# yjhuangcd/FI-ODE

Measured on AMD Instinct MI355X. Metric: CIFAR-10 train-step images/sec (B=128, h_sample=256) at 1/2/4/8 MI355X, higher is better.
Workload: dtype f32; 1 GPU; hipGraph replay: BASELINE configs[1]: train step of README.md:27 at epoch 20 with train_ode (rk4, step_size 0.1, t_max=1: 10 steps / 40 train-mode f-evals, backprop through the stages; loss_ode portion 0.2) + the Lyapunov loss (B=128, h_sample_size=256 -> 204 uniform + 52 correct-cone rows/image), KWLarge-Cayley backbone + Adam; global_batch=128, h_sample_size=256, rows_per_rank=32768, parallelism=dp1

## Files before the change

### fi-ode_amd/csrc/sconv.hip

```cpp
#include <hip/hip_runtime.h>
#include <stdint.h>

#include "common.h"
#include "fft.h"
#include "fiode.h"

namespace {

typedef float2 c32;
constexpr int BT_F = 16;
constexpr int BT_I = 8;
#ifndef SCONV_NTF8
#define SCONV_NTF8 512
#endif
#ifndef SCONV_NTF16
#define SCONV_NTF16 512
#endif
#ifndef SCONV_NTF32
#define SCONV_NTF32 512
#endif
#ifndef SCONV_NTF32S
#define SCONV_NTF32S 512
#endif
#ifndef SCONV_NTI8
// ... 37 lines not shown
  const c32* Y;
  const float* bias;
  float* y;
  uint8_t* code_out;
  const float* xn;
  const float* mu;
  const float* sd;
  const c32* Q;
  const c32* Xq;
};

__device__ __forceinline__ int64_t act_index(const SArgs& a, int h, int w, int c, int b) {
  return (((int64_t)h * a.n + w) * a.C + c) * a.B + b;
}
__device__ __forceinline__ int64_t nchw_index(const SArgs& a, int h, int w, int c, int b) {
  return (((int64_t)b * a.C + c) * a.n + h) * a.n + w;
}
__device__ __forceinline__ int64_t code_index(const SArgs& a, int h, int w, int c0, int b) {
  const int half = a.C >> 1;
  return a.nchw ? (((int64_t)b * half + c0) * a.n + h) * a.n + w : (((int64_t)h * a.n + w) * half + c0) * a.B + b;
}
__device__ __forceinline__ int64_t raw_index(const SArgs& a, int h, int w, int c, int b) {
  const int cr = c >> 2, dh = (c >> 1) & 1, dw = c & 1, C4 = a.C >> 2, n2 = 2 * a.n;
  return (((int64_t)(2 * h + dh) * n2 + (2 * w + dw)) * C4 + cr) * a.B + b;
}

constexpr int pad_is(int n, int bt, bool inv) {
  return inv ? (n == 8 ? 76 : n == 16 ? 276 : (bt == 4 ? 1064 : 1060))
             : n == 8 ? (bt == 4 ? 72 : 74) : n == 16 ? (bt == 4 ? 280 : 274)
                                                      : (bt == 4 ? 1064 : bt == 8 ? 1060 : 1058);
}
constexpr int pad_zs(int n, int bt, bool inv) {
  return inv ? (n == 8 ? 42 : n == 16 ? 146 : (bt == 4 ? 548 : 546))
             : n == 8 ? (bt == 4 ? 44 : 41) : n == 16 ? (bt == 4 ? 148 : 145)
                                                      : (bt == 4 ? 548 : bt == 8 ? 546 : 545);
}
template <int N, int BT, bool INV>
struct Geo {
  static constexpr int H = N / 2 + 1;
  static constexpr int RS = N + 1;
  static constexpr int IS = pad_is(N, BT, INV);
  static constexpr int ZS = pad_zs(N, BT, INV);
  static_assert(IS >= N * RS && ZS >= N * H, "image strides");
};

template <int N, int BT>
struct FGeo {
  typedef Geo<N, BT, false> g;
  static constexpr int H = g::H;
  static constexpr int ZS = g::ZS;
  static constexpr int CS = BT * ZS;
  static constexpr int NT = nthreads<N, BT, false>();
  __device__ static int pix(int ch, int bt, int h) { return 2 * (ch * CS + bt * ZS + h * H); }
};

template <int N, int BT, int NCH>
__device__ __forceinline__ void rfft2_inplace(const SArgs& a, int c0, int c1, int b0, c32* Z) {
  typedef FGeo<N, BT> G;
  constexpr int H = G::H, NT = G::NT;
  const float* img = reinterpret_cast<const float*>(Z);
  const int tid = threadIdx.x;
  for (int row = tid; row < NCH * BT * N; row += NT) {
    const int ch = row / (BT * N), r = row - ch * (BT * N);
    const int bt = r % BT, h = r / BT;
    const float* src = img + G::pix(ch, bt, h);
    c32 x[N];
#pragma unroll
    for (int w = 0; w < N; ++w) x[w] = make_float2(src[w], 0.f);
    fiode_fft::fft_reg<N, false>(x);
    c32* dst = Z + ch * G::CS + bt * G::ZS + h * H;
#pragma unroll
    for (int kb = 0; kb < H; ++kb) dst[kb] = x[kb];
  }
  __syncthreads();
  for (int col = tid; col < NCH * BT * H; col += NT) {
    const int ch = col / (BT * H), r = col - ch * (BT * H);
    const int bt = r % BT, kb = r / BT;
    const c32* cp = Z + ch * G::CS + bt * G::ZS + kb;
    c32 x[N];
#pragma unroll
    for (int h = 0; h < N; ++h) x[h] = cp[h * H];
    fiode_fft::fft_reg<N, false>(x);
    const int b = b0 + bt, c = ch ? c1 : c0;
    if (b < a.B) {
#pragma unroll
      for (int ka = 0; ka < N; ++ka) a.X[((int64_t)(ka * H + kb) * a.C + c) * a.B + b] = x[ka];
    }
  }
}

template <int N, int BT>
__global__ void __launch_bounds__((nthreads<N, BT, false>())) k_sconv_rfft2(SArgs a) {
  typedef FGeo<N, BT> G;
  constexpr int NT = G::NT;
  constexpr int NL = BT * N * N;
  constexpr int TR = (NL + NT - 1) / NT;
  __shared__ c32 Z[2 * G::CS];
  float* img = reinterpret_cast<float*>(Z);
  const int b0 = blockIdx.y * BT, tid = threadIdx.x;
  if (a.gy) {
    const int half = a.C >> 1, c0 = blockIdx.x, c1 = c0 + half;
#pragma unroll
    for (int t = 0; t < TR; ++t) {
      const int idx = tid + t * NT;
      if (idx < NL) {
        const int bt = a.nchw ? idx / (N * N) : idx % BT;
        const int hw = a.nchw ? idx % (N * N) : idx / BT, h = hw / N, w = hw % N;
        const int b = min(b0 + bt, a.B - 1);
        const uint8_t code = a.code[code_index(a, h, w, c0, b)];
        const float gmx = a.gy[a.nchw ? nchw_index(a, h, w, c0, b) : act_index(a, h, w, c0, b)];
        const float gmn = a.gy[a.nchw ? nchw_index(a, h, w, c1, b) : act_index(a, h, w, c1, b)];
        const bool in = b0 + bt < a.B;
        img[G::pix(0, bt, h) + w] = in ? gs_grad(gmx, gmn, code, true) : 0.f;
        img[G::pix(1, bt, h) + w] = in ? gs_grad(gmx, gmn, code, false) : 0.f;
      }
    }
// ... 12 lines not shown
        const int b = min(b0 + bt, a.B - 1);
        float v = a.xn[(((int64_t)b * a.C + c) * N + h) * N + w] - m;
        if (a.sd) v = v / sdv;
        img[G::pix(0, bt, h) + w] = b0 + bt < a.B ? v : 0.f;
      }
    }
  } else if (a.ds) {
#pragma unroll
    for (int t = 0; t < TR; ++t) {
      const int idx = tid + t * NT;
      if (idx < NL) {
        const int bt = idx % BT, hw = idx / BT, h = hw / N, w = hw % N;
        const int b = min(b0 + bt, a.B - 1);
        const float v = a.x[raw_index(a, h, w, c, b)];
        img[G::pix(0, bt, h) + w] = b0 + bt < a.B ? v : 0.f;
      }
    }
  } else {
#pragma unroll
    for (int t = 0; t < TR; ++t) {
      const int idx = tid + t * NT;
      if (idx < NL) {
        const int bt = idx % BT, hw = idx / BT, h = hw / N, w = hw % N;
        const int b = min(b0 + bt, a.B - 1);
        const float v = a.x[act_index(a, h, w, c, b)];
        img[G::pix(0, bt, h) + w] = b0 + bt < a.B ? v : 0.f;
      }
    }
  }
  __syncthreads();
  rfft2_inplace<N, BT, 1>(a, c, c, b0, Z);
}

template <int N>
struct IGeo {
  typedef Geo<N, bt_inv<N>(), true> g;
  static constexpr int BTI = bt_inv<N>();
  static constexpr int H = g::H;
  static constexpr int ZS = g::ZS;
  static constexpr int CS = BTI * ZS;
  static constexpr int NT = nthreads<N, BTI, true>();
  __device__ static int pix(int ch, int bt, int h) { return 2 * (ch * CS + bt * ZS + h * H); }
};

template <int N, int NCH, int KQ>
__device__ __forceinline__ void irfft2_inplace(const SArgs& a, int c0, int c1, int b0, c32* Ys) {
  typedef IGeo<N> G;
  constexpr int BTI = G::BTI, H = G::H, NT = G::NT;
  constexpr int NL = NCH * BTI * N * H;
  constexpr int TR = (NL + NT - 1) / NT;
  const int tid = threadIdx.x;
  if constexpr (KQ == 0) {
#pragma unroll
    for (int t = 0; t < TR; ++t) {
      const int idx = tid + t * NT;
      if (idx < NL) {
        const int ch = idx / (BTI * N * H), r = idx - ch * (BTI * N * H);
        const int bt = r % BTI, f = r / BTI;
        const int b = min(b0 + bt, a.B - 1);
        const c32 v = a.Y[((int64_t)f * a.C + (ch ? c1 : c0)) * a.B + b];
        Ys[ch * G::CS + bt * G::ZS + f] = b0 + bt < a.B ? v : make_float2(0.f, 0.f);
      }
    }
  } else {
    constexpr int NL1 = BTI * N * H;
    constexpr int TR1 = (NL1 + NT - 1) / NT;
#pragma unroll
    for (int t = 0; t < TR1; ++t) {
      const int idx = tid + t * NT;
      if (idx < NL1) {
        const int bt = idx % BTI, f = idx / BTI;
        const int b = min(b0 + bt, a.B - 1);
        const c32* xq = a.Xq + (int64_t)f * KQ * a.B + b;
        c32 xk[KQ], qk[NCH][KQ];
#pragma unroll
        for (int k = 0; k < KQ; ++k) xk[k] = xq[(int64_t)k * a.B];
#pragma unroll
        for (int ch = 0; ch < NCH; ++ch) {
          const c32* q = a.Q + ((int64_t)f * a.C + (ch ? c1 : c0)) * KQ;
#pragma unroll
          for (int k = 0; k < KQ; ++k) qk[ch][k] = q[k];
        }
#pragma unroll
        for (int ch = 0; ch < NCH; ++ch) {
          c32 v = make_float2(0.f, 0.f);
#pragma unroll
          for (int k = 0; k < KQ; ++k) {
            v.x += qk[ch][k].x * xk[k].x - qk[ch][k].y * xk[k].y;
            v.y += qk[ch][k].x * xk[k].y + qk[ch][k].y * xk[k].x;
          }
          Ys[ch * G::CS + bt * G::ZS + f] = b0 + bt < a.B ? v : make_float2(0.f, 0.f);
        }
      }
// ... 44 lines not shown
  const int b0 = blockIdx.y * BTI, tid = threadIdx.x;
  if (a.gs) {
    const int half = a.C >> 1, c0 = blockIdx.x, c1 = c0 + half;
    irfft2_inplace<N, 2, KQ>(a, c0, c1, b0, Ys);
    const float bb0 = a.bias ? a.bias[c0] : 0.f, bb1 = a.bias ? a.bias[c1] : 0.f;
    for (int idx = tid; idx < BTI * N * N; idx += NT) {
      const int bt = a.nchw ? idx / (N * N) : idx % BTI;
      const int hw = a.nchw ? idx % (N * N) : idx / BTI, h = hw / N, w = hw % N;
      const int b = b0 + bt;
      if (b >= a.B) continue;
      const float p = o[G::pix(0, bt, h) + w] + bb0, q = o[G::pix(1, bt, h) + w] + bb1;
      a.y[a.nchw ? nchw_index(a, h, w, c0, b) : act_index(a, h, w, c0, b)] = fmaxf(p, q);
      a.y[a.nchw ? nchw_index(a, h, w, c1, b) : act_index(a, h, w, c1, b)] = fminf(p, q);
      a.code_out[code_index(a, h, w, c0, b)] = p > q ? GS_GT : (p < q ? GS_LT : GS_EQ);
    }
    (void)half;
  } else {
    const int c = blockIdx.x;
    irfft2_inplace<N, 1, KQ>(a, c, c, b0, Ys);
    const float bb = a.bias ? a.bias[c] : 0.f;
    for (int idx = tid; idx < BTI * N * N; idx += NT) {
      const int bt = a.nchw ? idx / (N * N) : idx % BTI;
      const int hw = a.nchw ? idx % (N * N) : idx / BTI, h = hw / N, w = hw % N;
      const int b = b0 + bt;
      if (b >= a.B) continue;
      const float v = o[G::pix(0, bt, h) + w] + bb;
      if (a.ds) a.y[raw_index(a, h, w, c, b)] = v;
      else if (a.nchw) a.y[nchw_index(a, h, w, c, b)] = v;
      else a.y[act_index(a, h, w, c, b)] = v;
    }
  }
}

int check(const fiode_sconv_config* cfg, SArgs& a) {
  if (!cfg) return FIODE_EINVAL;
  a = SArgs{};
  a.n = cfg->n;
  a.C = cfg->C;
  a.B = cfg->B;
  a.ds = cfg->downsample ? 1 : 0;
  a.nchw = cfg->nchw ? 1 : 0;
  if ((a.n != 8 && a.n != 16 && a.n != 32) || a.C < 1 || a.B < 1) return FIODE_ESHAPE;
  if (a.nchw && a.ds) return FIODE_ESHAPE;
  if (a.ds && (a.C & 3)) return FIODE_ESHAPE;
  a.H = a.n / 2 + 1;
  return FIODE_OK;
}

}

extern "C" int fiode_sconv_rfft2(void* stream, const fiode_sconv_config* cfg, const float* x, const float* gy,
                                 const uint8_t* code, void* X) {
  SArgs a;
  int rc = check(cfg, a);
  if (rc) return rc;
  if (!X || (!x && !gy) || (gy && (!code || (a.C & 1) || a.ds))) return FIODE_EINVAL;
  a.x = x;
  a.gy = gy;
  a.code = code;
  a.X = (c32*)X;
  hipStream_t st = (hipStream_t)stream;
  const bool small = (int64_t)a.C * ((a.B + BT_F - 1) / BT_F) < 256;
  const int bt = small ? 4 : a.n == 32 ? SCONV_BTF32 : BT_F;
  const dim3 grid(gy ? a.C / 2 : a.C, (a.B + bt - 1) / bt);
  if (a.n == 8) {
    if (small) hipLaunchKernelGGL((k_sconv_rfft2<8, 4>), grid, dim3(nthreads<8, 4, false>()), 0, st, a);
// ... 59 lines not shown
  a.bias = bias;
  a.y = y;
  a.code_out = code_out;
  return FIODE_OK;
}

}

extern "C" int fiode_sconv_irfft2(void* stream, const fiode_sconv_config* cfg, const void* Y, const float* bias,
                                  int32_t groupsort, float* y, uint8_t* code_out) {
  SArgs a;
  const int rc = irfft2_common(cfg, bias, groupsort, y, code_out, a);
  if (rc) return rc;
  if (!Y) return FIODE_EINVAL;
  a.Y = (const c32*)Y;
  const hipError_t e = launch_irfft2<0>(a, (hipStream_t)stream);
  return e == hipSuccess ? FIODE_OK : FIODE_EHIP + (int)e;
}

extern "C" int fiode_sconv_irfft2_qx(void* stream, const fiode_sconv_config* cfg, const void* Q, const void* X,
                                     int32_t K, const float* bias, int32_t groupsort, float* y, uint8_t* code_out) {
  SArgs a;
  const int rc = irfft2_common(cfg, bias, groupsort, y, code_out, a);
  if (rc) return rc;
  if (K < 1 || K > 4) return FIODE_ESHAPE;
  if (!Q || !X) return FIODE_EINVAL;
  a.Q = (const c32*)Q;
  a.Xq = (const c32*)X;
  hipStream_t st = (hipStream_t)stream;
  const hipError_t e = K == 1 ? launch_irfft2<1>(a, st) : K == 2 ? launch_irfft2<2>(a, st)
                     : K == 3 ? launch_irfft2<3>(a, st) : launch_irfft2<4>(a, st);
  return e == hipSuccess ? FIODE_OK : FIODE_EHIP + (int)e;
}
```

### fi-ode_amd/fiode_amd/_lib.py

```python
from __future__ import annotations

import ctypes as ct
import os
import pathlib

_HERE = pathlib.Path(__file__).resolve().parent
LIB_PATH = pathlib.Path(os.environ.get("FIODE_LIB", _HERE / "libfiode.so"))

FIODE_SAMPLER_GIVEN, FIODE_SAMPLER_COMPOSITE, FIODE_SAMPLER_DECISION_BOUNDARY, FIODE_SAMPLER_TRAJECTORY = 0, 1, 2, 3
FIODE_DROPOUT_OFF, FIODE_DROPOUT_GIVEN, FIODE_DROPOUT_PHILOX = 0, 1, 2
FIODE_ACT_RELU, FIODE_ACT_GROUPSORT = 0, 1

class FiodeLibraryError(RuntimeError):
    pass


class FiodeError(RuntimeError):
    pass


_fp = ct.POINTER(ct.c_float)
_vp = ct.c_void_p


# ... 166 lines not shown
        "fiode_ode_nll": (ct.c_int, [_vp, ct.c_int32, _vp, _vp, _vp, _vp]),
        "fiode_ode_loss_mix": (ct.c_int, [_vp, ct.c_int32, _vp, _vp, _vp, ct.c_float, _vp, _vp, _vp]),
        "fiode_small_cayley_forward": (ct.c_int, [_vp, ct.c_int32, ct.c_int32, ct.c_int32, _vp, _vp, _vp, _vp, _vp]),
        "fiode_small_cayley_backward": (ct.c_int, [_vp, ct.c_int32, ct.c_int32, ct.c_int32, _vp, _vp, _vp, _vp, _vp,
                                                   _vp, _vp]),
        "fiode_dense_cayley_prep": (ct.c_int, [_vp, ct.POINTER(DenseConfig), _vp, _vp, _vp, _vp, _vp]),
        "fiode_dense_norm_workspace_bytes": (ct.c_size_t, [ct.POINTER(DenseConfig)]),
        "fiode_dense_norm_partials": (ct.c_int, [_vp, ct.POINTER(DenseConfig), _vp, _vp, ct.c_size_t]),
        "fiode_dense_cayley_prep_normed": (ct.c_int, [_vp, ct.POINTER(DenseConfig), _vp, _vp, _vp, _vp, _vp, _vp]),
        "fiode_dense_norm_partials_clear": (ct.c_int, [_vp, ct.POINTER(DenseConfig), _vp, _vp, ct.c_size_t, _vp,
                                                       ct.c_size_t, ct.c_size_t]),
        "fiode_dense_inverse_flag_bytes": (ct.c_size_t, [ct.c_int32]),
        "fiode_dense_cayley_inverse": (ct.c_int, [_vp, ct.POINTER(DenseConfig), _vp, _vp, _vp, _vp, _vp, _vp, _vp,
                                                  _vp, ct.c_size_t]),
        "fiode_dense_cayley_finish": (ct.c_int, [_vp, ct.POINTER(DenseConfig), _vp, _vp, _vp, _vp, _vp]),
        "fiode_dense_cayley_ginv": (ct.c_int, [_vp, ct.POINTER(DenseConfig), _vp, _vp, _vp, _vp, _vp]),
        "fiode_dense_cayley_h": (ct.c_int, [_vp, ct.POINTER(DenseConfig), _vp, _vp, _vp]),
        "fiode_dense_cayley_workspace_bytes": (ct.c_size_t, [ct.POINTER(DenseConfig)]),
        "fiode_dense_cayley_grad": (ct.c_int, [_vp, ct.POINTER(DenseConfig), _vp, _vp, _vp, _vp, _vp, _vp, _vp, _vp,
                                               _vp, ct.c_size_t]),
        "fiode_dense_gemm": (ct.c_int, [_vp, ct.c_int32, ct.c_int32, ct.c_int32, ct.c_int32, _vp, _vp, _vp]),
        "fiode_gemm_splits": (ct.c_int32, [ct.POINTER(GemmDesc)]),
        "fiode_gemm_counter_bytes": (ct.c_size_t, [ct.POINTER(GemmDesc)]),
        "fiode_gemm_workspace_bytes": (ct.c_size_t, [ct.POINTER(GemmDesc)]),
        "fiode_gemm": (ct.c_int, [_vp, ct.POINTER(GemmDesc), _vp, _vp, _vp, _vp, _vp, ct.c_size_t]),
        "fiode_gemm_pair_workspace_bytes": (ct.c_size_t, [ct.POINTER(GemmDesc), ct.POINTER(GemmDesc)]),
        "fiode_gemm_pair": (ct.c_int, [_vp, ct.POINTER(GemmDesc), _vp, _vp, _vp, _vp, ct.POINTER(GemmDesc), _vp, _vp,
                                       _vp, _vp, _vp, ct.c_size_t]),
        "fiode_sconv_rfft2": (ct.c_int, [_vp, ct.POINTER(SconvConfig), _vp, _vp, _vp, _vp]),
        "fiode_sconv_irfft2": (ct.c_int, [_vp, ct.POINTER(SconvConfig), _vp, _vp, ct.c_int32, _vp, _vp]),
        "fiode_sconv_rfft2_nchw": (ct.c_int, [_vp, ct.POINTER(SconvConfig), _vp, _vp, _vp, _vp]),
        "fiode_sconv_irfft2_qx": (ct.c_int, [_vp, ct.POINTER(SconvConfig), _vp, _vp, ct.c_int32, _vp, ct.c_int32,
                                             _vp, _vp]),
        "fiode_cgemm": (ct.c_int, [_vp, ct.c_int32, ct.c_int32, ct.c_int32, ct.c_int32, ct.c_int32, ct.c_int32, _vp,
                                   _vp, _vp, _vp]),
        "fiode_spectral_workspace_bytes": (ct.c_size_t, [ct.POINTER(SpectralConfig)]),
        "fiode_spectral_cayley_forward": (ct.c_int, [_vp, ct.POINTER(SpectralConfig), _vp, _vp, _vp, _vp, _vp,
                                                     ct.c_size_t]),
        "fiode_spectral_cayley_backward": (ct.c_int, [_vp, ct.POINTER(SpectralConfig), _vp, _vp, _vp, _vp, _vp, _vp,
                                                      _vp, ct.c_size_t]),
        "fiode_adam_step": (ct.c_int, [_vp, ct.POINTER(AdamConfig), _vp, _vp, _vp, _vp, _vp, _vp,
                                       ct.POINTER(StepGuard)]),
        "fiode_step_guard_flag": (ct.c_int, [_vp, ct.POINTER(StepGuard), _vp]),
        "fiode_error_string": (ct.c_char_p, [ct.c_int]),
        "fiode_abi_version": (ct.c_int, []),
    }
    for name, (res, args) in sig.items():
        if not hasattr(lib, name) and "FIODE_LIB" in os.environ:
            continue
        fn = getattr(lib, name)
        fn.restype = res
        fn.argtypes = args
    return lib


_LIB = None


def lib():
    global _LIB
    if _LIB is None:
        lb = _load()
        v = lb.fiode_abi_version()
        if v != ABI_VERSION:
            raise FiodeLibraryError(f"{LIB_PATH}: ABI version {v}, this package binds {ABI_VERSION} "
                                    "(stale build: run `make -C fi-ode_amd/csrc`)")
# ... 9 lines not shown
```

### fi-ode_amd/fiode_amd/cayley.py

```python
from __future__ import annotations

import ctypes as ct
import math
from typing import Optional

import torch
import torch.nn as nn
import torch.nn.functional as F

from .streams import current, fork, join, prefetch, run_on, shared, take


_BLOCK = 128


def _block_inverse(M: torch.Tensor) -> torch.Tensor:
    from . import ops
    n = M.shape[-1]
    if n > 64 and M.dtype == torch.float32 and M.is_cuda:
        if M.dim() == 2:
            return ops.block_inverse(M)
        return ops.block_inverse(M.reshape(-1, n, n)).reshape(M.shape)
    if n <= _BLOCK:
        return ops.batched_inverse(M)
# ... 466 lines not shown
    @staticmethod
    def backward(ctx, gQ):
        from . import ops
        weight, alpha, inv, ws = ctx.saved_tensors
        gw, ga = ops.spectral_cayley_backward(gQ.contiguous(), weight.detach(), alpha.detach(), ctx.n, inv, ws)
        return gw, ga.reshape(alpha.shape), None


class _SpectralCayleyStoredFn(torch.autograd.Function):

    @staticmethod
    def forward(ctx, weight, alpha, n: int, store: dict):
        ctx.save_for_backward(weight, alpha)
        ctx.store, ctx.n = store, n
        return store["Q"].detach()

    @staticmethod
    def backward(ctx, gQ):
        from . import ops
        weight, alpha = ctx.saved_tensors
        st = ctx.store
        gw, ga = ops.spectral_cayley_backward(gQ.contiguous(), weight.detach(), alpha.detach(), ctx.n, st["inv"],
                                              st["ws"])
        ga = ga.reshape(alpha.shape)
        hook = st.get("on_grads")
        if hook is not None:
            hook(gw, ga)
        return gw, ga, None, None


class _SpectralConvFn(torch.autograd.Function):

    @staticmethod
    def forward(ctx, x, Q, bias, n: int, downsample: bool, groupsort: bool, norm=None, nchw_out: bool = False):
        from . import ops
        nf, cout, cin = Q.shape
        if norm is not None:
            B = x.shape[0]
            X = ops.sconv_rfft2_nchw(x.detach(), norm[0], norm[1], n)
        else:
            B = x.shape[-1]
            X = ops.sconv_rfft2(x.detach(), n, cin, B, downsample=downsample)
        bd = None if bias is None else bias.detach()
        if cin <= SCONV_QX_MAX_K and not downsample:
            y, code = ops.sconv_irfft2_qx(Q.detach(), X, n, B, bias=bd, groupsort=groupsort, nchw=nchw_out)
        else:
            y, code = ops.sconv_irfft2(ops.cgemm(Q.detach(), X), n, cout, B, bias=bd, groupsort=groupsort,
                                       nchw=nchw_out)
        ctx.save_for_backward(X, Q, code)
        ctx.cfg = (n, downsample, groupsort, bias is not None, cin, cout, B)
        ctx.nchw_out = nchw_out
        return y

    @staticmethod
    def backward(ctx, gy):
        from . import ops
        X, Q, code = ctx.saved_tensors
        n, downsample, groupsort, has_bias, cin, cout, B = ctx.cfg
        gy = gy.contiguous()
        if groupsort:
            G = ops.sconv_rfft2(None, n, cout, B, gy=gy, code=code, nchw=ctx.nchw_out)
        else:
            G = ops.sconv_rfft2(gy, n, cout, B)
        gx = gQ = gb = None
        need_x, need_q, need_b = ctx.needs_input_grad[0], ctx.needs_input_grad[1], has_bias and ctx.needs_input_grad[2]
        wq = None
        if need_q:
            key = (n, str(G.device))
            wq = _SPECTRAL_GRAD_WEIGHTS.get(key)
            if wq is None:
                kb = torch.arange(n // 2 + 1, device=G.device)
                w = torch.where((kb == 0) | (kb == n // 2), 1.0, 2.0) / float(n * n)
                wq = _SPECTRAL_GRAD_WEIGHTS[key] = w.repeat(n).reshape(-1, 1, 1)

        def wgrad():
            if need_q and CONV_WGRAD_LIB:
                gq = torch.matmul(G, X.mH) * wq
            else:
                gq = ops.cgemm(G, X, conj_trans_b=True, scale=wq.reshape(-1)) if need_q else None
            gbias = G[0].real.sum(-1) if need_b else None
            return gq, gbias
        side = _head_stream(G.device) if (G.is_cuda and need_x and (need_q or need_b)) else None
        branch = fork(side, wgrad, reads=(G, X))
        if need_x:
            gx, _ = ops.sconv_irfft2(_q_h_g(Q, G), n, cin, B, downsample=downsample)
        (gQ, gb), = join(branch)
        return gx, gQ, gb, None, None, None, None, None


_SPECTRAL_GRAD_WEIGHTS = {}
CONV_WGRAD_LIB = True
SCONV_QX_MAX_K = 4


def _q_h_g(Q, G):
    from . import ops
    return ops.cgemm(Q.detach(), G, conj_trans_a=True)




class CayleyConv(nn.Conv2d):

    def __init__(self, in_channels: int, out_channels: int, kernel_size: int, stride: int = 1, bias: bool = True):
        self.downsample = stride == 2
        super().__init__(in_channels * (4 if self.downsample else 1), out_channels, kernel_size, stride=1,
                         padding=kernel_size // 2, bias=bias)
        self.alpha = nn.Parameter(torch.ones(1))
        self._alpha_init = False
        self.fused = True
        self._fused_shapes = {}
        self._shift = {}
        self._n = None
        self._pre = None
        self._store = None

    def _load_from_state_dict(self, *args, **kw):
        super()._load_from_state_dict(*args, **kw)
        self._alpha_init = True

# ... 55 lines not shown
            n = self._n
            self._pre = prefetch(stream, lambda: self.spectral_weight(n, self.weight.device))

    def _take_spectral(self, n: int, device) -> torch.Tensor:
        st = self._store
        if st is not None and self.training and st["n"] == n and torch.is_grad_enabled():
            Q = run_on(current().conv_stream(self),
                       lambda: _SpectralCayleyStoredFn.apply(self.weight, self.alpha, n, st))
            self._pre = None
            return Q
        if self._pre is not None and self.training and self._n == n:
            Q = take(self._pre)
        else:
            Q = self.spectral_weight(n, device)
        self._pre = None
        self._n = n
        return Q

    def forward(self, x: torch.Tensor) -> torch.Tensor:
        if self.downsample:
            b, c, h, w = x.shape
            x = x.reshape(b, c, h // 2, 2, w // 2, 2).permute(0, 1, 3, 5, 2, 4).reshape(b, c * 4, h // 2, w // 2)
        cout, cin = self.weight.shape[:2]
        B, _, n, _ = x.shape
        nf = n * (n // 2 + 1)
        xf = torch.fft.rfft2(x).permute(2, 3, 1, 0).reshape(nf, cin, B)
        Q = self._take_spectral(n, x.device)
        yf = (Q @ xf).reshape(n, n // 2 + 1, cout, B)
        y = torch.fft.irfft2(yf.permute(3, 2, 0, 1), s=(n, n))
        if self.bias is not None:
            y = y + self.bias[:, None, None]
        return y

    def forward_hwcb_fused(self, x: torch.Tensor, groupsort: bool, nchw_out: bool = False) -> torch.Tensor:
        n = x.shape[0] // 2 if self.downsample else x.shape[0]
        Q = self._take_spectral(n, x.device)
        return _SpectralConvFn.apply(x, Q, self.bias, n, self.downsample, groupsort, None,
                                     bool(nchw_out and groupsort))

    def forward_nchw_fused(self, x: torch.Tensor, mu: torch.Tensor, sd, groupsort: bool) -> torch.Tensor:
        n = x.shape[-1]
        Q = self._take_spectral(n, x.device)
        return _SpectralConvFn.apply(x, Q, self.bias, n, False, groupsort, (mu, sd))

    def forward_hwcb(self, x: torch.Tensor) -> torch.Tensor:
        if self.downsample:
            h, w, c, b = x.shape
            x = x.reshape(h // 2, 2, w // 2, 2, c, b).permute(0, 2, 4, 1, 3, 5).reshape(h // 2, w // 2, c * 4, b)
        cout, cin = self.weight.shape[:2]
        n, _, _, B = x.shape
        nf = n * (n // 2 + 1)
        xf = torch.fft.rfft2(x, dim=(0, 1)).reshape(nf, cin, B)
        Q = self._take_spectral(n, x.device)
        yf = Q @ xf
        if self.bias is not None:
            yf[0] += (float(n * n) * self.bias)[:, None]
        return torch.fft.irfft2(yf.reshape(n, n // 2 + 1, cout, B), s=(n, n), dim=(0, 1))
```

### fi-ode_amd/fiode_amd/models.py

```python
from __future__ import annotations

from typing import Optional, Sequence

import torch
import torch.nn as nn

from .cayley import CayleyConv, CayleyLinear, GroupSort, linear_head


class Normalize(nn.Module):

    def __init__(self, mu: Sequence[float], std: Optional[Sequence[float]]):
        super().__init__()
        self.register_buffer("mu", torch.tensor(list(mu), dtype=torch.float32).view(-1, 1, 1))
        self.register_buffer("std", None if std is None else torch.tensor(list(std), dtype=torch.float32).view(-1, 1, 1))

    fused_hwcb = True

    def forward(self, x):
        if self.fused_hwcb and x.is_cuda and x.dtype == torch.float32 and x.dim() == 4 and not x.requires_grad:
            from . import _lib as L, ops
            B, C, H, W = x.shape
            xc = x.contiguous()
            y = torch.empty((H, W, C, B), dtype=torch.float32, device=x.device)
            mu = self.mu.reshape(-1).contiguous()
            sd = None if self.std is None else self.std.reshape(-1).contiguous()
            L.check(L.lib().fiode_normalize_hwcb(ops._stream(x.device), B, C, H, W, xc.data_ptr(), mu.data_ptr(),
                                                 None if sd is None else sd.data_ptr(), y.data_ptr()),
                    "fiode_normalize_hwcb")
            return y.permute(3, 2, 0, 1)
        if self.std is not None:
            return (x - self.mu) / self.std
        return x - self.mu


class KWLargeConcat(nn.Module):

    def __init__(self, out_dim: int = 10, act: str = "GroupSort", w: int = 1):
        super().__init__()
        act_fn = GroupSort if act == "GroupSort" else nn.ReLU
        self.model = nn.Sequential(
            CayleyConv(3, 32 * w, 3), act_fn(),
            CayleyConv(32 * w, 32 * w, 3, stride=2), act_fn(),
            CayleyConv(32 * w, 64 * w, 3), act_fn(),
            CayleyConv(64 * w, 64 * w, 3, stride=2), act_fn(),
            nn.Flatten(),
            CayleyLinear(4096 * w, 512 * w), act_fn(),
            CayleyLinear(512 * w, 512), act_fn(),
            CayleyLinear(512, out_dim),
        )

        self.spatial_major = True
        self.fused_transforms = True
        self.nchw_last = True

    def can_take_nchw(self, x) -> bool:
        m = self.model[0]
        return (self.spatial_major and self.fused_transforms and x.is_cuda and x.dtype == torch.float32
                and x.dim() == 4 and not x.requires_grad and isinstance(m, CayleyConv) and not m.downsample
                and x.shape[-1] == x.shape[-2] and x.shape[-1] in (8, 16, 32))

    def forward(self, x, norm=None):
        if not (self.spatial_major and x.is_cuda):
            return self.model(x)
        mods = list(self.model)
        i = 0
        nconv = 0
        if norm is not None:
            if getattr(self, "after_conv_hook", None) is not None:
                self.after_conv_hook(-1)
            gs = isinstance(mods[1], GroupSort)
            h = mods[0].forward_nchw_fused(x, norm[0], norm[1], gs)
            i = 2 if gs else 1
            if getattr(self, "after_conv_hook", None) is not None:
                self.after_conv_hook(0)
            nconv = 1
        else:
            h = x.permute(2, 3, 1, 0).contiguous()
            if getattr(self, "after_conv_hook", None) is not None:
                self.after_conv_hook(-1)
        nchw = False
        while not isinstance(mods[i], nn.Flatten):
            m = mods[i]
            if isinstance(m, CayleyConv):
                gs = i + 1 < len(mods) and isinstance(mods[i + 1], GroupSort)
                if self.fused_transforms and h.shape[0] // (2 if m.downsample else 1) <= 32:
                    nchw = bool(self.nchw_last and gs and i + 2 < len(mods) and isinstance(mods[i + 2], nn.Flatten))
                    h = m.forward_hwcb_fused(h, gs, nchw_out=nchw)
                    i += 2 if gs else 1
                    if getattr(self, "after_conv_hook", None) is not None:
                        self.after_conv_hook(nconv)
                    nconv += 1
                    continue
                h = m.forward_hwcb(h)
                if getattr(self, "after_conv_hook", None) is not None:
                    self.after_conv_hook(nconv)
                nconv += 1
            elif isinstance(m, GroupSort):
                h = m(h, channel_dim=2)
            else:
                h = m(h)
            i += 1
        h = h.reshape(h.shape[0], -1) if nchw else h.permute(3, 2, 0, 1).reshape(h.shape[3], -1)
        return linear_head(mods[i + 1:], h)


class NormalizedBackbone(nn.Sequential):

    fused_input = True

    def forward(self, x):
        norm, net = self[0], self[1]
        if (self.fused_input and len(self) == 2 and isinstance(norm, Normalize) and isinstance(net, KWLargeConcat)
                and norm.fused_hwcb and net.can_take_nchw(x)):
            return net(x.contiguous(), norm=(norm.mu, norm.std))
        return super().forward(x)


def make_ortho_KWLarge_Concat(n_in_channels=3, n_outputs=10, mu=(0.485, 0.456, 0.406), std=(0.225, 0.225, 0.225),
                              out_dim=10, act="GroupSort"):
    return NormalizedBackbone(Normalize(mu, std), KWLargeConcat(out_dim=out_dim, act=act))
# ... 45 lines not shown
```

### fi-ode_amd/fiode_amd/ops.py

```python
from __future__ import annotations

import ctypes as ct
from dataclasses import dataclass
from typing import Dict, Optional

import torch

from . import _lib as L

C, M, X = 10, 128, 10
WEIGHT_KEYS = ("Q1", "b1", "Qx", "bx", "Q2", "b2", "Q3", "b3")
WEIGHT_SHAPES = {"Q1": (M, C), "b1": (M,), "Qx": (M, X), "bx": (M,), "Q2": (M, M), "b2": (M,),
                 "Q3": (C, M), "b3": (C,)}


@dataclass
class DynCfg:
    alpha_1: float = 100.0
    alpha_2: float = 20.0
    sigma_1: float = 0.02
    scale_nominal: bool = True
    dropout: float = 0.5
    qp_max_iter: int = 30
    qp_tol: float = 1e-4
# ... 638 lines not shown
        bias = _need(bias.detach(), "bias", (C,), torch.float32, dev)
    if nchw and downsample:
        raise ValueError("sconv_irfft2: nchw and downsample together")
    shape = (2 * n, 2 * n, C // 4, B) if downsample else ((B, C, n, n) if nchw else (n, n, C, B))
    y = torch.empty(shape, dtype=torch.float32, device=dev)
    code = (torch.empty((B, C // 2, n, n) if nchw else (n, n, C // 2, B), dtype=torch.uint8, device=dev)
            if groupsort else None)
    cfg = L.SconvConfig(n, C, B, int(bool(downsample)), int(bool(nchw)))
    L.check(L.lib().fiode_sconv_irfft2(_stream(dev), ct.byref(cfg), Y.data_ptr(), _ptr(bias), int(bool(groupsort)),
                                       y.data_ptr(), _ptr(code)), "fiode_sconv_irfft2")
    return y, code


def sconv_irfft2_qx(Q: torch.Tensor, X: torch.Tensor, n: int, B: int, bias: Optional[torch.Tensor] = None,
                    groupsort: bool = False, nchw: bool = False):
    dev = X.device
    nf = n * (n // 2 + 1)
    if Q.dim() != 3 or Q.shape[0] != nf:
        raise ValueError(f"sconv_irfft2_qx: Q {tuple(Q.shape)} is not [{nf}, C, K]")
    C, K = Q.shape[1], Q.shape[2]
    Q = _need(Q.detach(), "Q", (nf, C, K), torch.complex64, dev)
    X = _need(X.detach(), "X", (nf, K, B), torch.complex64, dev)
    if bias is not None:
        bias = _need(bias.detach(), "bias", (C,), torch.float32, dev)
    y = torch.empty((B, C, n, n) if nchw else (n, n, C, B), dtype=torch.float32, device=dev)
    code = (torch.empty((B, C // 2, n, n) if nchw else (n, n, C // 2, B), dtype=torch.uint8, device=dev)
            if groupsort else None)
    cfg = L.SconvConfig(n, C, B, 0, int(bool(nchw)))
    L.check(L.lib().fiode_sconv_irfft2_qx(_stream(dev), ct.byref(cfg), Q.data_ptr(), X.data_ptr(), K, _ptr(bias),
                                          int(bool(groupsort)), y.data_ptr(), _ptr(code)), "fiode_sconv_irfft2_qx")
    return y, code


def cgemm(A: torch.Tensor, B: torch.Tensor, conj_trans_a: bool = False, conj_trans_b: bool = False,
          scale: Optional[torch.Tensor] = None) -> torch.Tensor:
    dev = B.device
    if A.dim() != 3 or B.dim() != 3 or A.dtype != torch.complex64 or B.dtype != torch.complex64:
        raise ValueError(f"cgemm: complex64 [F, ., .] operands, got {tuple(A.shape)} {A.dtype}, "
                         f"{tuple(B.shape)} {B.dtype}")
    if conj_trans_a and conj_trans_b:
        raise ValueError("cgemm: conj_trans_a and conj_trans_b together are not supported")
    F = B.shape[0]
    K, N = (B.shape[2], B.shape[1]) if conj_trans_b else (B.shape[1], B.shape[2])
    M, ka = (A.shape[2], A.shape[1]) if conj_trans_a else (A.shape[1], A.shape[2])
    if A.shape[0] != F or ka != K or A.device != dev:
        raise ValueError(f"cgemm: A {tuple(A.shape)} does not match B {tuple(B.shape)}")
    if scale is not None:
        scale = _need(scale.detach().reshape(-1), "scale", (F,), torch.float32, dev)
    A = A.contiguous()
    B = B.contiguous()
    C = torch.empty((F, M, N), dtype=torch.complex64, device=dev)
    L.check(L.lib().fiode_cgemm(_stream(dev), F, M, N, K, int(bool(conj_trans_a)), int(bool(conj_trans_b)),
                                _ptr(scale), A.data_ptr(), B.data_ptr(), C.data_ptr()), "fiode_cgemm")
    return C


def _mat_layout(X: torch.Tensor):
    R, Cn = X.shape[-2], X.shape[-1]
    s0, s1 = X.stride(-2), X.stride(-1)
    if (s1 == 1 or Cn == 1) and (s0 >= Cn or R == 1):
        return 0, max(s0 if R > 1 else Cn, Cn, 1)
    if (s0 == 1 or R == 1) and (s1 >= R or Cn == 1):
        return 1, max(s1 if Cn > 1 else R, R, 1)
    return None


# ... 208 lines not shown
```

### include/fiode.h

```cpp
#ifndef FIODE_H_
#define FIODE_H_

#include <stddef.h>
#include <stdint.h>

#ifdef __cplusplus
extern "C" {
#endif

#define FIODE_ABI_VERSION 5

#if defined(__GNUC__)
#define FIODE_API __attribute__((visibility("default")))
#else
#define FIODE_API
#endif

enum {
  FIODE_OK = 0,
  FIODE_EINVAL = 1,
  FIODE_ESHAPE = 2,
  FIODE_EWORKSPACE = 3,
  FIODE_EHIP = 100
};
// ... 261 lines not shown
  int32_t trans_a, trans_b;
  int64_t lda, ldb, ldc;
  int64_t stride_a, stride_b, stride_c;
  float alpha, beta;
  int32_t split_k;
  int32_t max_workgroups;
} fiode_gemm_desc;
FIODE_API int32_t fiode_gemm_splits(const fiode_gemm_desc* d);
FIODE_API size_t fiode_gemm_counter_bytes(const fiode_gemm_desc* d);
FIODE_API size_t fiode_gemm_workspace_bytes(const fiode_gemm_desc* d);
FIODE_API int fiode_gemm(void* stream, const fiode_gemm_desc* d, const float* A, const float* B, const float* bias,
                         float* C, void* workspace, size_t workspace_bytes);
FIODE_API size_t fiode_gemm_pair_workspace_bytes(const fiode_gemm_desc* d0, const fiode_gemm_desc* d1);
FIODE_API int fiode_gemm_pair(void* stream, const fiode_gemm_desc* d0, const float* A0, const float* B0,
                              const float* bias0, float* C0, const fiode_gemm_desc* d1, const float* A1,
                              const float* B1, const float* bias1, float* C1, void* workspace,
                              size_t workspace_bytes);

typedef struct fiode_sconv_config {
  int32_t n;
  int32_t C;
  int32_t B;
  int32_t downsample;
  int32_t nchw;
} fiode_sconv_config;
FIODE_API int fiode_sconv_rfft2(void* stream, const fiode_sconv_config* cfg, const float* x, const float* gy,
                                const uint8_t* code, void* X);
FIODE_API int fiode_sconv_rfft2_nchw(void* stream, const fiode_sconv_config* cfg, const float* x, const float* mu,
                                     const float* std, void* X);
FIODE_API int fiode_sconv_irfft2(void* stream, const fiode_sconv_config* cfg, const void* Y, const float* bias,
                                 int32_t groupsort, float* y, uint8_t* code_out);
FIODE_API int fiode_sconv_irfft2_qx(void* stream, const fiode_sconv_config* cfg, const void* Q, const void* X,
                                    int32_t K, const float* bias, int32_t groupsort, float* y, uint8_t* code_out);

FIODE_API int fiode_cgemm(void* stream, int32_t F, int32_t M, int32_t N, int32_t K, int32_t conj_trans_a,
                          int32_t conj_trans_b, const float* scale, const void* A, const void* B, void* C);

typedef struct fiode_spectral_config {
  int32_t cout, cin;
  int32_t ks;
  int32_t n;
} fiode_spectral_config;

FIODE_API size_t fiode_spectral_workspace_bytes(const fiode_spectral_config* cfg);
FIODE_API int fiode_spectral_cayley_forward(void* stream, const fiode_spectral_config* cfg, const float* weight,
                                            const float* alpha, void* Q, void* inv, void* workspace,
                                            size_t workspace_bytes);
FIODE_API int fiode_spectral_cayley_backward(void* stream, const fiode_spectral_config* cfg, const float* weight,
                                             const float* alpha, const void* gQ, const void* inv,
                                             float* grad_weight, float* grad_alpha, void* workspace,
                                             size_t workspace_bytes);

#define FIODE_ADAM_MAX_TENSORS 64
#define FIODE_GUARD_MAX_STATUS 4
typedef struct fiode_step_guard {
  const float* flag;
  const float* loss;
  const int32_t* status[FIODE_GUARD_MAX_STATUS];
  int32_t* skipped;
} fiode_step_guard;
FIODE_API int fiode_step_guard_flag(void* stream, const fiode_step_guard* guard, float* flag_out);

typedef struct fiode_adam_config {
  int32_t n_tensors;
  int32_t decoupled;
  int32_t maximize;
// ... 19 lines not shown
```

Baseline: 105,900 images/s.

## Fuse irfft2+GroupSort+next-layer rfft2 at spectral conv boundaries

Adds boundary kernels that take one layer's spectral output, run the inverse FFT, bias and GroupSort, then apply the next layer's forward FFT (optionally with a space-to-depth downsample) in a single kernel, keeping activations in the spectral domain between consecutive Cayley convs. A matching backward kernel fuses irfft2 of the incoming gradient, the GroupSort gradient and the rfft2. The model's forward path routes eligible conv/GroupSort/conv chains through these kernels, and the backward pass skips the spatial transform when the input was already spectral. This removes the spatial-domain activation round trips through global memory and some launches, at the cost of heavier shared-memory kernels with new tile sizes and more complex autograd plumbing.

```diff
diff --git a/fi-ode_amd/csrc/sconv.hip b/fi-ode_amd/csrc/sconv.hip
--- a/fi-ode_amd/csrc/sconv.hip
+++ b/fi-ode_amd/csrc/sconv.hip
@@ -93,7 +93,7 @@
 }
 constexpr int pad_zs(int n, int bt, bool inv) {
   return inv ? (n == 8 ? 42 : n == 16 ? 146 : (bt == 4 ? 548 : 546))
-             : n == 8 ? (bt == 4 ? 44 : 41) : n == 16 ? (bt == 4 ? 148 : 145)
+             : n == 8 ? (bt == 4 ? 44 : bt == 8 ? 42 : 41) : n == 16 ? (bt == 4 ? 148 : bt == 8 ? 154 : 145)
                                                       : (bt == 4 ? 548 : bt == 8 ? 546 : 545);
 }
 template <int N, int BT, bool INV>
@@ -115,10 +115,16 @@
   __device__ static int pix(int ch, int bt, int h) { return 2 * (ch * CS + bt * ZS + h * H); }
 };
 
-template <int N, int BT, int NCH>
+template <int NCH>
+__device__ __forceinline__ int slot_channel(int ch, int c0, int c1) {
+  if constexpr (NCH > 2) return 4 * ((ch >> 2) ? c1 : c0) + (ch & 3);
+  else return ch ? c1 : c0;
+}
+
+template <int N, int BT, int NCH, int NT_ = 0>
 __device__ __forceinline__ void rfft2_inplace(const SArgs& a, int c0, int c1, int b0, c32* Z) {
   typedef FGeo<N, BT> G;
-  constexpr int H = G::H, NT = G::NT;
+  constexpr int H = G::H, NT = NT_ ? NT_ : G::NT;
   const float* img = reinterpret_cast<const float*>(Z);
   const int tid = threadIdx.x;
   for (int row = tid; row < NCH * BT * N; row += NT) {
@@ -142,7 +148,7 @@
 #pragma unroll
     for (int h = 0; h < N; ++h) x[h] = cp[h * H];
     fiode_fft::fft_reg<N, false>(x);
-    const int b = b0 + bt, c = ch ? c1 : c0;
+    const int b = b0 + bt, c = slot_channel<NCH>(ch, c0, c1);
     if (b < a.B) {
 #pragma unroll
       for (int ka = 0; ka < N; ++ka) a.X[((int64_t)(ka * H + kb) * a.C + c) * a.B + b] = x[ka];
@@ -221,10 +227,10 @@
   rfft2_inplace<N, BT, 1>(a, c, c, b0, Z);
 }
 
-template <int N>
+template <int N, int BTI_ = bt_inv<N>()>
 struct IGeo {
-  typedef Geo<N, bt_inv<N>(), true> g;
-  static constexpr int BTI = bt_inv<N>();
+  typedef Geo<N, BTI_, true> g;
+  static constexpr int BTI = BTI_;
   static constexpr int H = g::H;
   static constexpr int ZS = g::ZS;
   static constexpr int CS = BTI * ZS;
@@ -232,10 +238,10 @@
   __device__ static int pix(int ch, int bt, int h) { return 2 * (ch * CS + bt * ZS + h * H); }
 };
 
-template <int N, int NCH, int KQ>
+template <int N, int NCH, int KQ, int BTI_ = bt_inv<N>(), int NT_ = 0>
 __device__ __forceinline__ void irfft2_inplace(const SArgs& a, int c0, int c1, int b0, c32* Ys) {
-  typedef IGeo<N> G;
-  constexpr int BTI = G::BTI, H = G::H, NT = G::NT;
+  typedef IGeo<N, BTI_> G;
+  constexpr int BTI = G::BTI, H = G::H, NT = NT_ ? NT_ : G::NT;
   constexpr int NL = NCH * BTI * N * H;
   constexpr int TR = (NL + NT - 1) / NT;
   const int tid = threadIdx.x;
@@ -247,7 +253,7 @@
         const int ch = idx / (BTI * N * H), r = idx - ch * (BTI * N * H);
         const int bt = r % BTI, f = r / BTI;
         const int b = min(b0 + bt, a.B - 1);
-        const c32 v = a.Y[((int64_t)f * a.C + (ch ? c1 : c0)) * a.B + b];
+        const c32 v = a.Y[((int64_t)f * a.C + slot_channel<NCH>(ch, c0, c1)) * a.B + b];
         Ys[ch * G::CS + bt * G::ZS + f] = b0 + bt < a.B ? v : make_float2(0.f, 0.f);
       }
     }
@@ -358,6 +364,101 @@
   }
 }
 
+#ifndef SCONV_BTB
+#define SCONV_BTB 8
+#endif
+#ifndef SCONV_NTB8
+#define SCONV_NTB8 256
+#endif
+constexpr int BT_B = SCONV_BTB;
+#ifndef SCONV_BTB32F
+#define SCONV_BTB32F 4
+#endif
+#ifndef SCONV_BTB32B
+#define SCONV_BTB32B 8
+#endif
+#ifndef SCONV_NTB32F
+#define SCONV_NTB32F 512
+#endif
+
+template <int N, int KQ, bool DS, int BT, int NT>
+__global__ void __launch_bounds__(NT) k_sconv_fwd_boundary(SArgs a, SArgs f) {
+  constexpr int N2 = DS ? N / 2 : N, NCH2 = DS ? 8 : 2;
+  typedef IGeo<N, BT> IG;
+  typedef FGeo<N2, BT> FG;
+  __shared__ c32 Ys[2 * IG::CS];
+  __shared__ c32 Z[NCH2 * FG::CS];
+  const float* o = reinterpret_cast<const float*>(Ys);
+  float* img = reinterpret_cast<float*>(Z);
+  const int b0 = blockIdx.y * BT, tid = threadIdx.x;
+  const int c0 = blockIdx.x, c1 = c0 + (a.C >> 1);
+  irfft2_inplace<N, 2, KQ, BT, NT>(a, c0, c1, b0, Ys);
+  const float bb0 = a.bias ? a.bias[c0] : 0.f, bb1 = a.bias ? a.bias[c1] : 0.f;
+  for (int idx = tid; idx < BT * N * N; idx += NT) {
+    const int bt = idx % BT, hw = idx / BT, h = hw / N, w = hw % N;
+    const int b = b0 + bt;
+    const float p = o[IG::pix(0, bt, h) + w] + bb0, q = o[IG::pix(1, bt, h) + w] + bb1;
+    if (b < a.B) a.code_out[code_index(a, h, w, c0, b)] = p > q ? GS_GT : (p < q ? GS_LT : GS_EQ);
+    if constexpr (DS) {
+      const int sub = 2 * (h & 1) + (w & 1);
+      img[FG::pix(sub, bt, h >> 1) + (w >> 1)] = fmaxf(p, q);
+      img[FG::pix(4 + sub, bt, h >> 1) + (w >> 1)] = fminf(p, q);
+    } else {
+      img[FG::pix(0, bt, h) + w] = fmaxf(p, q);
+      img[FG::pix(1, bt, h) + w] = fminf(p, q);
+    }
+  }
+  __syncthreads();
+  rfft2_inplace<N2, BT, NCH2, NT>(f, c0, c1, b0, Z);
+}
+
+template <int N, bool DS, int BT, int NT>
+__global__ void __launch_bounds__(NT) k_sconv_bwd_boundary(SArgs a, SArgs g) {
+  constexpr int N2 = DS ? 2 * N : N, NCH = DS ? 8 : 2;
+  typedef IGeo<N, BT> IG;
+  typedef FGeo<N2, BT> FG;
+  constexpr int NL = BT * N2 * N2;
+  constexpr int TR = (NL + NT - 1) / NT;
+  __shared__ c32 Ys[NCH * IG::CS];
+  __shared__ c32 Z[2 * FG::CS];
+  const float* o = reinterpret_cast<const float*>(Ys);
+  float* img = reinterpret_cast<float*>(Z);
+  const int b0 = blockIdx.y * BT, tid = threadIdx.x;
+  const int c0 = blockIdx.x, c1 = c0 + (g.C >> 1);
+  uint8_t cd[TR];
+#pragma unroll
+  for (int t = 0; t < TR; ++t) {
+    const int idx = tid + t * NT;
+    cd[t] = GS_EQ;
+    if (idx < NL) {
+      const int bt = idx % BT, hw = idx / BT, h = hw / N2, w = hw % N2;
+      cd[t] = g.code[code_index(g, h, w, c0, min(b0 + bt, g.B - 1))];
+    }
+  }
+  irfft2_inplace<N, NCH, 0, BT, NT>(a, c0, c1, b0, Ys);
+#pragma unroll
+  for (int t = 0; t < TR; ++t) {
+    const int idx = tid + t * NT;
+    if (idx < NL) {
+      const int bt = idx % BT, hw = idx / BT, h = hw / N2, w = hw % N2;
+      float gmx, gmn;
+      if constexpr (DS) {
+        const int sub = 2 * (h & 1) + (w & 1);
+        gmx = o[IG::pix(sub, bt, h >> 1) + (w >> 1)] + 0.f;
+        gmn = o[IG::pix(4 + sub, bt, h >> 1) + (w >> 1)] + 0.f;
+      } else {
+        gmx = o[IG::pix(0, bt, h) + w] + 0.f;
+        gmn = o[IG::pix(1, bt, h) + w] + 0.f;
+      }
+      const bool in = b0 + bt < g.B;
+      img[FG::pix(0, bt, h) + w] = in ? gs_grad(gmx, gmn, cd[t], true) : 0.f;
+      img[FG::pix(1, bt, h) + w] = in ? gs_grad(gmx, gmn, cd[t], false) : 0.f;
+    }
+  }
+  __syncthreads();
+  rfft2_inplace<N2, BT, 2, NT>(g, c0, c1, b0, Z);
+}
+
 int check(const fiode_sconv_config* cfg, SArgs& a) {
   if (!cfg) return FIODE_EINVAL;
   a = SArgs{};
@@ -483,3 +584,75 @@
                      : K == 3 ? launch_irfft2<3>(a, st) : launch_irfft2<4>(a, st);
   return e == hipSuccess ? FIODE_OK : FIODE_EHIP + (int)e;
 }
+
+namespace {
+
+int boundary_args(const fiode_sconv_config* cfg, SArgs& a, SArgs& nx) {
+  if (!cfg) return FIODE_EINVAL;
+  fiode_sconv_config c = *cfg;
+  c.downsample = 0;
+  int rc = check(&c, a);
+  if (rc) return rc;
+  if (a.nchw || (a.C & 1)) return FIODE_ESHAPE;
+  nx = a;
+  if (cfg->downsample) {
+    nx.n = a.n / 2;
+    nx.H = nx.n / 2 + 1;
+    nx.C = 4 * a.C;
+  }
+  return FIODE_OK;
+}
+
+}
+
+extern "C" int fiode_sconv_boundary_fwd(void* stream, const fiode_sconv_config* cfg, const void* Y, const void* Q,
+                                        const void* Xq, int32_t K, const float* bias, uint8_t* code_out,
+                                        void* X_next) {
+  SArgs a, f;
+  int rc = boundary_args(cfg, a, f);
+  if (rc) return rc;
+  const bool ds = cfg->downsample != 0;
+  const bool qx = Y == nullptr;
+  if (qx && (K < 1 || K > 4)) return FIODE_ESHAPE;
+  const int kq = qx ? K : 0;
+  const bool ok = (a.n == 32 && ds && kq == 3) || (a.n == 16 && kq == 0);
+  if (!ok) return FIODE_ESHAPE;
+  if (!code_out || !X_next || (qx && (!Q || !Xq))) return FIODE_EINVAL;
+  a.Y = (const c32*)Y;
+  a.Q = (const c32*)Q;
+  a.Xq = (const c32*)Xq;
+  a.bias = bias;
+  a.code_out = code_out;
+  a.gs = 1;
+  f.X = (c32*)X_next;
+  hipStream_t st = (hipStream_t)stream;
+  const int bt = a.n == 32 ? SCONV_BTB32F : BT_B;
+  const dim3 grid(a.C / 2, (a.B + bt - 1) / bt);
+  if (a.n == 32) hipLaunchKernelGGL((k_sconv_fwd_boundary<32, 3, true, SCONV_BTB32F, SCONV_NTB32F>), grid, dim3(SCONV_NTB32F), 0, st, a, f);
+  else if (ds) hipLaunchKernelGGL((k_sconv_fwd_boundary<16, 0, true, BT_B, 512>), grid, dim3(512), 0, st, a, f);
+  else hipLaunchKernelGGL((k_sconv_fwd_boundary<16, 0, false, BT_B, 512>), grid, dim3(512), 0, st, a, f);
+  const hipError_t e = hipGetLastError();
+  return e == hipSuccess ? FIODE_OK : FIODE_EHIP + (int)e;
+}
+
+extern "C" int fiode_sconv_boundary_bwd(void* stream, const fiode_sconv_config* cfg, const void* M,
+                                        const uint8_t* code, void* G) {
+  SArgs g, a;
+  int rc = boundary_args(cfg, g, a);
+  if (rc) return rc;
+  const bool ds = cfg->downsample != 0;
+  const bool ok = ds ? (g.n == 16 || g.n == 32) : g.n == 16;
+  if (!ok) return FIODE_ESHAPE;
+  if (!M || !code || !G) return FIODE_EINVAL;
+  a.Y = (const c32*)M;
+  g.code = code;
+  g.X = (c32*)G;
+  hipStream_t st = (hipStream_t)stream;
+  const int bt = g.n == 32 ? SCONV_BTB32B : BT_B;
+  const dim3 grid(g.C / 2, (g.B + bt - 1) / bt);
+  if (g.n == 32) hipLaunchKernelGGL((k_sconv_bwd_boundary<16, true, SCONV_BTB32B, 512>), grid, dim3(512), 0, st, a, g);
+  else if (ds) hipLaunchKernelGGL((k_sconv_bwd_boundary<8, true, BT_B, SCONV_NTB8>), grid, dim3(SCONV_NTB8), 0, st, a, g);
+  else hipLaunchKernelGGL((k_sconv_bwd_boundary<16, false, BT_B, 512>), grid, dim3(512), 0, st, a, g);
+  const hipError_t e = hipGetLastError();
+  return e == hipSuccess ? FIODE_OK : FIODE_EHIP + (int)e;
+}
diff --git a/fi-ode_amd/fiode_amd/_lib.py b/fi-ode_amd/fiode_amd/_lib.py
--- a/fi-ode_amd/fiode_amd/_lib.py
+++ b/fi-ode_amd/fiode_amd/_lib.py
@@ -222,6 +222,9 @@
         "fiode_sconv_rfft2_nchw": (ct.c_int, [_vp, ct.POINTER(SconvConfig), _vp, _vp, _vp, _vp]),
         "fiode_sconv_irfft2_qx": (ct.c_int, [_vp, ct.POINTER(SconvConfig), _vp, _vp, ct.c_int32, _vp, ct.c_int32,
                                              _vp, _vp]),
+        "fiode_sconv_boundary_fwd": (ct.c_int, [_vp, ct.POINTER(SconvConfig), _vp, _vp, _vp, ct.c_int32, _vp, _vp,
+                                                _vp]),
+        "fiode_sconv_boundary_bwd": (ct.c_int, [_vp, ct.POINTER(SconvConfig), _vp, _vp, _vp]),
         "fiode_cgemm": (ct.c_int, [_vp, ct.c_int32, ct.c_int32, ct.c_int32, ct.c_int32, ct.c_int32, ct.c_int32, _vp,
                                    _vp, _vp, _vp]),
         "fiode_spectral_workspace_bytes": (ct.c_size_t, [ct.POINTER(SpectralConfig)]),
diff --git a/fi-ode_amd/fiode_amd/cayley.py b/fi-ode_amd/fiode_amd/cayley.py
--- a/fi-ode_amd/fiode_amd/cayley.py
+++ b/fi-ode_amd/fiode_amd/cayley.py
@@ -522,17 +522,29 @@
 class _SpectralConvFn(torch.autograd.Function):
 
     @staticmethod
-    def forward(ctx, x, Q, bias, n: int, downsample: bool, groupsort: bool, norm=None, nchw_out: bool = False):
+    def forward(ctx, x, Q, bias, n: int, downsample: bool, groupsort: bool, norm=None, nchw_out: bool = False,
+                spec_in: bool = False, boundary=None):
         from . import ops
         nf, cout, cin = Q.shape
-        if norm is not None:
+        if spec_in:
+            B = x.shape[-1]
+            X = x.detach()
+        elif norm is not None:
             B = x.shape[0]
             X = ops.sconv_rfft2_nchw(x.detach(), norm[0], norm[1], n)
         else:
             B = x.shape[-1]
             X = ops.sconv_rfft2(x.detach(), n, cin, B, downsample=downsample)
         bd = None if bias is None else bias.detach()
-        if cin <= SCONV_QX_MAX_K and not downsample:
+        qx = cin <= SCONV_QX_MAX_K and not downsample
+        if boundary is not None:
+            if qx:
+                y, code = ops.sconv_boundary_fwd(None, n, cout, B, bias=bd, downsample_next=boundary, Q=Q.detach(),
+                                                 X=X)
+            else:
+                y, code = ops.sconv_boundary_fwd(ops.cgemm(Q.detach(), X), n, cout, B, bias=bd,
+                                                 downsample_next=boundary)
+        elif qx:
             y, code = ops.sconv_irfft2_qx(Q.detach(), X, n, B, bias=bd, groupsort=groupsort, nchw=nchw_out)
         else:
             y, code = ops.sconv_irfft2(ops.cgemm(Q.detach(), X), n, cout, B, bias=bd, groupsort=groupsort,
@@ -540,6 +552,7 @@
         ctx.save_for_backward(X, Q, code)
         ctx.cfg = (n, downsample, groupsort, bias is not None, cin, cout, B)
         ctx.nchw_out = nchw_out
+        ctx.spec_in, ctx.boundary = spec_in, boundary
         return y
 
     @staticmethod
@@ -548,7 +561,9 @@
         X, Q, code = ctx.saved_tensors
         n, downsample, groupsort, has_bias, cin, cout, B = ctx.cfg
         gy = gy.contiguous()
-        if groupsort:
+        if ctx.boundary is not None:
+            G = ops.sconv_boundary_bwd(gy, code, n, cout, B, downsample_next=ctx.boundary)
+        elif groupsort:
             G = ops.sconv_rfft2(None, n, cout, B, gy=gy, code=code, nchw=ctx.nchw_out)
         else:
             G = ops.sconv_rfft2(gy, n, cout, B)
@@ -573,9 +588,12 @@
         side = _head_stream(G.device) if (G.is_cuda and need_x and (need_q or need_b)) else None
         branch = fork(side, wgrad, reads=(G, X))
         if need_x:
-            gx, _ = ops.sconv_irfft2(_q_h_g(Q, G), n, cin, B, downsample=downsample)
+            if ctx.spec_in:
+                gx = _q_h_g(Q, G)
+            else:
+                gx, _ = ops.sconv_irfft2(_q_h_g(Q, G), n, cin, B, downsample=downsample)
         (gQ, gb), = join(branch)
-        return gx, gQ, gb, None, None, None, None, None
+        return gx, gQ, gb, None, None, None, None, None, None, None
 
 
 _SPECTRAL_GRAD_WEIGHTS = {}
@@ -697,16 +715,28 @@
             y = y + self.bias[:, None, None]
         return y
 
-    def forward_hwcb_fused(self, x: torch.Tensor, groupsort: bool, nchw_out: bool = False) -> torch.Tensor:
-        n = x.shape[0] // 2 if self.downsample else x.shape[0]
+    def forward_hwcb_fused(self, x: torch.Tensor, groupsort: bool, nchw_out: bool = False, spec_n=None,
+                           boundary=None) -> torch.Tensor:
+        if spec_n is not None:
+            n = spec_n
+        else:
+            n = x.shape[0] // 2 if self.downsample else x.shape[0]
         Q = self._take_spectral(n, x.device)
         return _SpectralConvFn.apply(x, Q, self.bias, n, self.downsample, groupsort, None,
-                                     bool(nchw_out and groupsort))
-
-    def forward_nchw_fused(self, x: torch.Tensor, mu: torch.Tensor, sd, groupsort: bool) -> torch.Tensor:
+                                     bool(nchw_out and groupsort), spec_n is not None, boundary)
+
+    def boundary_ok(self, n: int, nxt: "CayleyConv") -> bool:
+        from . import ops
+        cout, cin = self.weight.shape[:2]
+        K = cin if (cin <= SCONV_QX_MAX_K and not self.downsample) else 0
+        return (cout % 2 == 0 and nxt.weight.shape[1] == cout * (4 if nxt.downsample else 1)
+                and (n, nxt.downsample, K) in ops.SCONV_BOUNDARIES_FWD
+                and (n, nxt.downsample) in ops.SCONV_BOUNDARIES_BWD)
+
+    def forward_nchw_fused(self, x: torch.Tensor, mu: torch.Tensor, sd, groupsort: bool, boundary=None) -> torch.Tensor:
         n = x.shape[-1]
         Q = self._take_spectral(n, x.device)
-        return _SpectralConvFn.apply(x, Q, self.bias, n, False, groupsort, (mu, sd))
+        return _SpectralConvFn.apply(x, Q, self.bias, n, False, groupsort, (mu, sd), False, False, boundary)
 
     def forward_hwcb(self, x: torch.Tensor) -> torch.Tensor:
         if self.downsample:
diff --git a/fi-ode_amd/fiode_amd/models.py b/fi-ode_amd/fiode_amd/models.py
--- a/fi-ode_amd/fiode_amd/models.py
+++ b/fi-ode_amd/fiode_amd/models.py
@@ -54,6 +54,14 @@
         self.fused_transforms = True
         self.nchw_last = True
 
+    fused_boundaries = True
+
+    def _boundary(self, mods, i: int, n: int):
+        if not (self.fused_boundaries and self.fused_transforms and i + 2 < len(mods)
+                and isinstance(mods[i + 1], GroupSort) and isinstance(mods[i + 2], CayleyConv)):
+            return None
+        return bool(mods[i + 2].downsample) if mods[i].boundary_ok(n, mods[i + 2]) else None
+
     def can_take_nchw(self, x) -> bool:
         m = self.model[0]
         return (self.spatial_major and self.fused_transforms and x.is_cuda and x.dtype == torch.float32
@@ -66,11 +74,15 @@
         mods = list(self.model)
         i = 0
         nconv = 0
+        spec_n = None
         if norm is not None:
             if getattr(self, "after_conv_hook", None) is not None:
                 self.after_conv_hook(-1)
             gs = isinstance(mods[1], GroupSort)
-            h = mods[0].forward_nchw_fused(x, norm[0], norm[1], gs)
+            bnd = self._boundary(mods, 0, x.shape[-1])
+            h = mods[0].forward_nchw_fused(x, norm[0], norm[1], gs, boundary=bnd)
+            if bnd is not None:
+                spec_n = x.shape[-1] // 2 if bnd else x.shape[-1]
             i = 2 if gs else 1
             if getattr(self, "after_conv_hook", None) is not None:
                 self.after_conv_hook(0)
@@ -84,9 +96,12 @@
             m = mods[i]
             if isinstance(m, CayleyConv):
                 gs = i + 1 < len(mods) and isinstance(mods[i + 1], GroupSort)
-                if self.fused_transforms and h.shape[0] // (2 if m.downsample else 1) <= 32:
+                n = spec_n if spec_n is not None else h.shape[0] // (2 if m.downsample else 1)
+                if self.fused_transforms and n <= 32:
                     nchw = bool(self.nchw_last and gs and i + 2 < len(mods) and isinstance(mods[i + 2], nn.Flatten))
-                    h = m.forward_hwcb_fused(h, gs, nchw_out=nchw)
+                    bnd = self._boundary(mods, i, n) if gs else None
+                    h = m.forward_hwcb_fused(h, gs, nchw_out=nchw, spec_n=spec_n, boundary=bnd)
+                    spec_n = None if bnd is None else (n // 2 if bnd else n)
                     i += 2 if gs else 1
                     if getattr(self, "after_conv_hook", None) is not None:
                         self.after_conv_hook(nconv)
diff --git a/fi-ode_amd/fiode_amd/ops.py b/fi-ode_amd/fiode_amd/ops.py
--- a/fi-ode_amd/fiode_amd/ops.py
+++ b/fi-ode_amd/fiode_amd/ops.py
@@ -694,6 +694,49 @@
     return y, code
 
 
+SCONV_BOUNDARIES_FWD = ((32, True, 3), (16, False, 0), (16, True, 0))
+SCONV_BOUNDARIES_BWD = ((16, True), (16, False), (32, True))
+
+
+def sconv_boundary_fwd(Y: Optional[torch.Tensor], n: int, C: int, B: int, bias: Optional[torch.Tensor] = None,
+                       downsample_next: bool = False, Q: Optional[torch.Tensor] = None,
+                       X: Optional[torch.Tensor] = None):
+    nf = n * (n // 2 + 1)
+    K = 0
+    if Y is not None:
+        dev = Y.device
+        Y = _need(Y, "Y", (nf, C, B), torch.complex64, dev)
+    else:
+        dev = X.device
+        if Q.dim() != 3 or Q.shape[0] != nf or Q.shape[1] != C:
+            raise ValueError(f"sconv_boundary_fwd: Q {tuple(Q.shape)} is not [{nf}, {C}, K]")
+        K = Q.shape[2]
+        Q = _need(Q.detach(), "Q", (nf, C, K), torch.complex64, dev)
+        X = _need(X.detach(), "X", (nf, K, B), torch.complex64, dev)
+    if bias is not None:
+        bias = _need(bias.detach(), "bias", (C,), torch.float32, dev)
+    n2, C2 = (n // 2, 4 * C) if downsample_next else (n, C)
+    Xn = torch.empty((n2 * (n2 // 2 + 1), C2, B), dtype=torch.complex64, device=dev)
+    code = torch.empty((n, n, C // 2, B), dtype=torch.uint8, device=dev)
+    cfg = L.SconvConfig(n, C, B, int(bool(downsample_next)), 0)
+    L.check(L.lib().fiode_sconv_boundary_fwd(_stream(dev), ct.byref(cfg), _ptr(Y), _ptr(Q), _ptr(X), K, _ptr(bias),
+                                             code.data_ptr(), Xn.data_ptr()), "fiode_sconv_boundary_fwd")
+    return Xn, code
+
+
+def sconv_boundary_bwd(M: torch.Tensor, code: torch.Tensor, n: int, C: int, B: int,
+                       downsample_next: bool = False) -> torch.Tensor:
+    dev = M.device
+    n2, C2 = (n // 2, 4 * C) if downsample_next else (n, C)
+    M = _need(M, "M", (n2 * (n2 // 2 + 1), C2, B), torch.complex64, dev)
+    code = _need(code, "code", (n, n, C // 2, B), torch.uint8, dev)
+    G = torch.empty((n * (n // 2 + 1), C, B), dtype=torch.complex64, device=dev)
+    cfg = L.SconvConfig(n, C, B, int(bool(downsample_next)), 0)
+    L.check(L.lib().fiode_sconv_boundary_bwd(_stream(dev), ct.byref(cfg), M.data_ptr(), code.data_ptr(),
+                                             G.data_ptr()), "fiode_sconv_boundary_bwd")
+    return G
+
+
 def cgemm(A: torch.Tensor, B: torch.Tensor, conj_trans_a: bool = False, conj_trans_b: bool = False,
           scale: Optional[torch.Tensor] = None) -> torch.Tensor:
     dev = B.device
diff --git a/include/fiode.h b/include/fiode.h
--- a/include/fiode.h
+++ b/include/fiode.h
@@ -317,6 +317,11 @@
                                  int32_t groupsort, float* y, uint8_t* code_out);
 FIODE_API int fiode_sconv_irfft2_qx(void* stream, const fiode_sconv_config* cfg, const void* Q, const void* X,
                                     int32_t K, const float* bias, int32_t groupsort, float* y, uint8_t* code_out);
+FIODE_API int fiode_sconv_boundary_fwd(void* stream, const fiode_sconv_config* cfg, const void* Y, const void* Q,
+                                       const void* Xq, int32_t K, const float* bias, uint8_t* code_out,
+                                       void* X_next);
+FIODE_API int fiode_sconv_boundary_bwd(void* stream, const fiode_sconv_config* cfg, const void* M,
+                                       const uint8_t* code, void* G);
 
 FIODE_API int fiode_cgemm(void* stream, int32_t F, int32_t M, int32_t N, int32_t K, int32_t conj_trans_a,
                           int32_t conj_trans_b, const float* scale, const void* A, const void* B, void* C);
```

Measured after the change: 108,100 images/s, median of 6. About the same (+2.1%).
